# zeehu/generative_ranking_recommender

Measured on AMD Instinct MI355X. Metric: vectors quantized/sec (3-level RQ, 512-d), higher is better.
Workload: dtype f32

## Files before the change

generative_ranking_recommender_amd/csrc/assign_common.h:

```cpp
#pragma once
#include <cmath>
#include <cstdlib>
#include <type_traits>

#include "assign_plan.h"
#include "internal.h"

#ifndef RQSID_AB_MODE
#define RQSID_AB_MODE 0
#endif

namespace rqsid {

typedef __attribute__((ext_vector_type(8))) _Float16 f16x8;
typedef __attribute__((ext_vector_type(2))) _Float16 h2;
typedef __attribute__((ext_vector_type(2))) float f2;
typedef __attribute__((ext_vector_type(16))) float f32x16;

constexpr int kWaves = 4;
constexpr int kRowsPerWave = 32;
constexpr int kTileRows = kWaves * kRowsPerWave;
constexpr int kChunk = 32;
constexpr int kXWaveBytes = kRowsPerWave * 128;
constexpr int kXStage = kWaves * kXWaveBytes;
// ... 117 lines not shown
__device__ __forceinline__ void dma16_nt_off(const void* gsrc, uint32_t lds_base) {
  uint32_t keep;
  asm volatile(
      RQ_M0_SAVE
      "s_mov_b32 m0, %2\n\t"
      "s_nop 0\n\t"
      "global_load_lds_dwordx4 %1, off offset:%3 nt"
      RQ_M0_RESTORE
      : "=&s"(keep)
      : "v"(gsrc), "s"(lds_base), "i"(OFF)
      : "memory");
}
__device__ __forceinline__ void dma16_nt(const void* gsrc, uint32_t lds_base) {
  uint32_t keep;
  asm volatile(
      RQ_M0_SAVE
      "s_mov_b32 m0, %2\n\t"
      "s_nop 0\n\t"
      "global_load_lds_dwordx4 %1, off nt"
      RQ_M0_RESTORE
      : "=&s"(keep)
      : "v"(gsrc), "s"(lds_base)
      : "memory");
}

__device__ __forceinline__ void dma16_r(const void* gsrc, uint32_t lds_base) {
  uint32_t keep;
  asm volatile(
      RQ_M0_SAVE
      "s_mov_b32 m0, %2\n\t"
      "s_nop 0\n\t"
      "global_load_lds_dwordx4 %1, off"
      RQ_M0_RESTORE
      : "=&s"(keep)
      : "v"(gsrc), "s"(lds_base));
}
__device__ __forceinline__ void dma16_nt_r(const void* gsrc, uint32_t lds_base) {
  uint32_t keep;
  asm volatile(
      RQ_M0_SAVE
      "s_mov_b32 m0, %2\n\t"
      "s_nop 0\n\t"
      "global_load_lds_dwordx4 %1, off nt"
      RQ_M0_RESTORE
      : "=&s"(keep)
      : "v"(gsrc), "s"(lds_base));
}
#define RQSID_PIN_MFMA() __builtin_amdgcn_sched_barrier(0x0106)

template <int N>
__device__ __forceinline__ void wait_barrier() {
  asm volatile("s_waitcnt vmcnt(%0)\n\ts_waitcnt lgkmcnt(0)\n\ts_barrier" ::"i"(N) : "memory");
}

template <int S, int P>
__device__ __forceinline__ void wait_chunks(int younger) {
  static_assert((S - 2) * P <= 63, "vmcnt field is 6 bits");
  if (S >= 7 && younger >= 5) wait_barrier<(S >= 7 ? 5 * P : 0)>();
  else if (S >= 6 && younger >= 4) wait_barrier<(S >= 6 ? 4 * P : 0)>();
  else if (S >= 5 && younger >= 3) wait_barrier<(S >= 5 ? 3 * P : 0)>();
  else if (S >= 4 && younger >= 2) wait_barrier<(S >= 4 ? 2 * P : 0)>();
  else if (younger >= 1) wait_barrier<P>();
  else wait_barrier<0>();
}

__device__ __forceinline__ int xor32(int x) {
  const auto sw = __builtin_amdgcn_permlane32_swap((unsigned)x, (unsigned)x, false, false);
  return (int)((threadIdx.x & 32) ? sw[0] : sw[1]);
}
__device__ __forceinline__ float xor32(float x) { return __int_as_float(xor32(__float_as_int(x))); }
__device__ __forceinline__ double xor32(double x) {
  const uint64_t u = (uint64_t)__double_as_longlong(x);
  const uint64_t lo = (uint32_t)xor32((int)(uint32_t)u), hi = (uint32_t)xor32((int)(uint32_t)(u >> 32));
  return __longlong_as_double((long long)((hi << 32) | lo));
}

__device__ __forceinline__ void push_work(const AssignParams& p, bool need, int lane, const WorkItem& w) {
  const unsigned long long m = __ballot(need);
  if (!m) return;
  const int leader = __ffsll((long long)m) - 1;
  int base = 0;
  if (lane == leader) base = atomicAdd(p.work_count, __popcll(m));
  base = __shfl(base, leader);
  if (need) {
    const int idx = base + __popcll(m & ((1ull << lane) - 1ull));
    if (idx < p.work_cap) p.work[idx] = w;
  }
}

constexpr double kTrunc = 16.0;
inline float accumulation_rel(int dim) {
  return (float)((kTrunc + (dim / 16) / 2.0 + 1.0) * std::ldexp(1.0, -23) * 1.02);
}

template <int NW>
__device__ __forceinline__ int pass_take_first(uint32_t (&wv)[NW], int h) {
  int ws = -1;
  uint32_t b = 0;
#pragma unroll
  for (int w = NW - 1; w >= 0; --w) {
    const bool nz = wv[w] != 0;
    ws = nz ? w : ws;
    b = nz ? wv[w] : b;
  }
  const int jj = __clz(b) & 31;
  const int t = 2 * ws + (jj >> 4), v = jj & 15;
  const int k = ws >= 0 ? t * 32 + (v & 3) + 8 * (v >> 2) + 4 * h : -1;
#pragma unroll
  for (int w = 0; w < NW; ++w) wv[w] = w == ws ? (wv[w] & ~(0x80000000u >> jj)) : wv[w];
  return k;
}

template <int NW>
__device__ __forceinline__ bool pass_decide(const uint32_t (&pbits)[NW], int h, int& k_out, WorkItem& w) {
  int pc = 0;
#pragma unroll
  for (int i = 0; i < NW; ++i) pc += __popc(pbits[i]);
  const int pc_o = xor32(pc);
  const int ncand = pc + pc_o;
  const bool overflow = pc > kListPerHalf || pc_o > kListPerHalf || ncand == 0;
  const bool definitive = !overflow && ncand == 1;
  uint32_t wv[NW];
#pragma unroll
  for (int i = 0; i < NW; ++i) wv[i] = pbits[i];
  const int k0 = pass_take_first(wv, h);
  k_out = max(k0, xor32(k0));
  w.n = overflow ? -1 : ncand;
  if (__builtin_amdgcn_ballot_w64(!definitive && !overflow)) {
    int kk[kListPerHalf];
    kk[0] = k0;
#pragma unroll
    for (int j = 1; j < kListPerHalf; ++j) kk[j] = pass_take_first(wv, h);
    int c8[kMaxList];
#pragma unroll
    for (int j = 0; j < kListPerHalf; ++j) {
      const int o = xor32(kk[j]);
      c8[j] = kk[j] >= 0 ? kk[j] : INT_MAX;
      c8[kListPerHalf + j] = o >= 0 ? o : INT_MAX;
    }
#pragma unroll
    for (int i = 0; i < kMaxList; ++i)
#pragma unroll
      for (int j = 0; j < kMaxList - 1 - i; ++j) {
        const int a = c8[j], bq = c8[j + 1];
        c8[j] = min(a, bq);
        c8[j + 1] = max(a, bq);
      }
#pragma unroll
    for (int j = 0; j < kMaxList; ++j) w.cand[j] = (uint16_t)(c8[j] == INT_MAX ? 0xFFFF : c8[j]);
  }
  return definitive;
}

__device__ __forceinline__ float ratio_up(float num, float den) {
  return den > 0.f ? num / den * 1.000001f : (num > 0.f ? INFINITY : 0.f);
}
__device__ __forceinline__ float wave_max(float v) {
#pragma unroll
  for (int o = 32; o > 0; o >>= 1) v = fmaxf(v, __shfl_xor(v, o));
  return v;
}

#ifdef RQSID_STAMPS
#define ST_NOW() __builtin_amdgcn_s_memtime()
#define ST(x) x
#else
#define ST(x)
#endif

#ifndef RQSID_PACKED_MAIN
#define RQSID_PACKED_MAIN 0
#endif

constexpr int kErrSlot = 60;
constexpr int kErrCompact = 1;
constexpr int kErrOvfList = 2;
constexpr int kErrWorkIdx = 4;
constexpr int kErrTiles = 8;

struct RowSums {
  f2 se2v = {0.f, 0.f};
  f2 se2l = {0.f, 0.f};
  f2 sf2v = {0.f, 0.f};
  double sv2 = 0.0;
  double sv2b = 0.0;
};
constexpr bool fp64_norm(int rl, bool norm) { return norm && rl == 1; }

template <int HI>
__device__ __forceinline__ float sub_f16(float v, h2 hh) {
  float d;
  if (HI)
    asm("v_fma_mix_f32 %0, -%1, 1.0, %2 op_sel:[1,0,0] op_sel_hi:[1,0,0]" : "=v"(d) : "v"(hh), "v"(v));
  else
    asm("v_fma_mix_f32 %0, -%1, 1.0, %2 op_sel:[0,0,0] op_sel_hi:[1,0,0]" : "=v"(d) : "v"(hh), "v"(v));
  return d;
}

template <int XF, bool INFNAN>
__device__ __forceinline__ void widen2(uint32_t w, float& lo, float& hi) {
  static_assert(XF == RQSID_X_F16 || XF == RQSID_X_BF16, "16-bit row formats");
  if (XF == RQSID_X_BF16) {
    lo = __uint_as_float(w << 16);
    hi = __uint_as_float(w & 0xFFFF0000u);
  } else {
    const uint32_t sl = w << 16;
    uint32_t al = (w << 13) & 0x0FFFE000u, ah = (w >> 3) & 0x0FFFE000u;
    float fl = __uint_as_float(al) * 0x1p112f, fh = __uint_as_float(ah) * 0x1p112f;
    if (INFNAN) {
      fl = al >= 0x0F800000u ? __uint_as_float(__float_as_uint(fl) | 0x7F800000u) : fl;
      fh = ah >= 0x0F800000u ? __uint_as_float(__float_as_uint(fh) | 0x7F800000u) : fh;
    }
    lo = __uint_as_float((__float_as_uint(fl) & 0x7FFFFFFFu) | (sl & 0x80000000u));
    hi = __uint_as_float((__float_as_uint(fh) & 0x7FFFFFFFu) | (w & 0x80000000u));
  }
}
template <int XF>
__device__ __forceinline__ float4 load_row4(const float* x, int64_t row, int dim, int i) {
  if constexpr (XF == RQSID_X_F32) {
    return reinterpret_cast<const float4*>(x + row * dim)[i];
  } else {
    const uint2 w = reinterpret_cast<const uint2*>(reinterpret_cast<const uint16_t*>(x) + row * dim)[i];
    float4 a;
    widen2<XF, true>(w.x, a.x, a.y);
    widen2<XF, true>(w.y, a.z, a.w);
    return a;
  }
}

template <int RL, bool NORM, bool T3, bool SUMS>
__device__ __forceinline__ void row_frag(const float4 xa, const float4 xc, const float* lds_ca, const float* lds_cb,
                                         int d0, float inv1, f16x8& bf, f16x8& bl, RowSums& s) {
#if RQSID_PACKED_MAIN
  f2 v[4] = {f2{xa.x, xa.y}, f2{xa.z, xa.w}, f2{xc.x, xc.y}, f2{xc.z, xc.w}};
  if (RL >= 1) {
    const float4 a0 = *reinterpret_cast<const float4*>(lds_ca + d0);
    const float4 a1 = *reinterpret_cast<const float4*>(lds_ca + d0 + 4);
    const f2 av[4] = {f2{a0.x, a0.y}, f2{a0.z, a0.w}, f2{a1.x, a1.y}, f2{a1.z, a1.w}};
#pragma unroll
    for (int e = 0; e < 4; ++e) v[e] = v[e] - av[e];
  }
  if (RL >= 2) {
    const float4 b0 = *reinterpret_cast<const float4*>(lds_cb + d0);
    const float4 b1 = *reinterpret_cast<const float4*>(lds_cb + d0 + 4);
    const f2 bv[4] = {f2{b0.x, b0.y}, f2{b0.z, b0.w}, f2{b1.x, b1.y}, f2{b1.z, b1.w}};
#pragma unroll
    for (int e = 0; e < 4; ++e) v[e] = (NORM ? v[e] * inv1 : v[e]) - bv[e];
  }
  h2 hh[4], lh[4];
#pragma unroll
  for (int e = 0; e < 4; ++e) hh[e] = __builtin_convertvector(v[e], h2);
  bf = __builtin_shufflevector(__builtin_shufflevector(hh[0], hh[1], 0, 1, 2, 3),
                               __builtin_shufflevector(hh[2], hh[3], 0, 1, 2, 3), 0, 1, 2, 3, 4, 5, 6, 7);
  if (T3) {
#pragma unroll
    for (int e = 0; e < 4; ++e) {
      const f2 xs = (v[e] - __builtin_convertvector(hh[e], f2)) * 4096.0f;
      lh[e] = __builtin_convertvector(xs, h2);
      if (SUMS) {
        const f2 ev = xs - __builtin_convertvector(lh[e], f2);
        s.se2l = ev * ev + s.se2l;
      }
    }
    bl = __builtin_shufflevector(__builtin_shufflevector(lh[0], lh[1], 0, 1, 2, 3),
                                 __builtin_shufflevector(lh[2], lh[3], 0, 1, 2, 3), 0, 1, 2, 3, 4, 5, 6, 7);
  }
  if (SUMS) {
#pragma unroll
    for (int e = 0; e < 4; ++e) {
      const f2 ex = v[e] - __builtin_convertvector(hh[e], f2);
      s.se2v = ex * ex + s.se2v;
      if (fp64_norm(RL, NORM)) {
        s.sv2 = fma((double)v[e].x, (double)v[e].x, s.sv2);
        s.sv2b = fma((double)v[e].y, (double)v[e].y, s.sv2b);
      } else {
        s.sf2v = v[e] * v[e] + s.sf2v;
      }
    }
  }
#else
  float v[8] = {xa.x, xa.y, xa.z, xa.w, xc.x, xc.y, xc.z, xc.w};
  if (RL >= 1) {
    const float4 a0 = *reinterpret_cast<const float4*>(lds_ca + d0);
    const float4 a1 = *reinterpret_cast<const float4*>(lds_ca + d0 + 4);
    const float a[8] = {a0.x, a0.y, a0.z, a0.w, a1.x, a1.y, a1.z, a1.w};
#pragma unroll
    for (int e = 0; e < 8; ++e) v[e] = v[e] - a[e];
  }
  if (RL >= 2) {
    const float4 b0 = *reinterpret_cast<const float4*>(lds_cb + d0);
    const float4 b1 = *reinterpret_cast<const float4*>(lds_cb + d0 + 4);
    const float b[8] = {b0.x, b0.y, b0.z, b0.w, b1.x, b1.y, b1.z, b1.w};
#pragma unroll
    for (int e = 0; e < 8; ++e) v[e] = (NORM ? v[e] * inv1 : v[e]) - b[e];
  }
  h2 hh[4], lh[4];
#pragma unroll
  for (int e = 0; e < 4; ++e) hh[e] = __builtin_convertvector(f2{v[2 * e], v[2 * e + 1]}, h2);
  bf = __builtin_shufflevector(__builtin_shufflevector(hh[0], hh[1], 0, 1, 2, 3),
                               __builtin_shufflevector(hh[2], hh[3], 0, 1, 2, 3), 0, 1, 2, 3, 4, 5, 6, 7);
  float ex[8];
#pragma unroll
  for (int e = 0; e < 8; ++e) ex[e] = (e & 1) ? sub_f16<1>(v[e], hh[e >> 1]) : sub_f16<0>(v[e], hh[e >> 1]);
  if (T3) {
#pragma unroll
    for (int e = 0; e < 4; ++e) lh[e] = __builtin_convertvector(f2{ex[2 * e] * 4096.0f, ex[2 * e + 1] * 4096.0f}, h2);
// ... 99 lines not shown
```

generative_ranking_recommender_amd/csrc/assign_pc.hip:

```cpp
#define RQ_M0_KEEP 0
#include "assign_common.h"

#ifdef RQSID_STAMPS
__device__ unsigned long long g_pc_stamps[24];
#define PST(...) __VA_ARGS__
#define PNOW() __builtin_amdgcn_s_memtime()
#else
#define PST(...)
#endif

namespace rqsid {
namespace {

constexpr int kQDim = 512, kQC = 32, kQNch = kQDim / kQC;
constexpr int kQRows = 128;
constexpr int kQSentinel = -2;

struct PcDesc {
  int32_t s, t0, nrows, cnt, cbase, flags, ca_row, cb_row;
};
static_assert(sizeof(PcDesc) == 32, "descriptor layout");
static_assert(kQDim == kPlanPcDim && kQRows == kPlanPcRows && sizeof(PcDesc) == kPlanPcDescBytes, "assign_plan.h constants");

template <int NT, int RL, bool T3>
struct PcLayout {
  static constexpr int Sr = 4, Sc = 3;
  static constexpr int kTerms = T3 ? 2 : 1;
  static constexpr int kXS = kQRows * kQC * 4;
  static constexpr int kCT = NT * 32 * kQC * 2;
  static constexpr int kCS = kCT * kTerms;
  static constexpr int kBW = 2 * kTerms * 1024;
  static constexpr int kBS = 4 * kBW;
  static constexpr int kX = 0;
  static constexpr int kC = kX + Sr * kXS;
  static constexpr int kB = kC + Sc * kCS;
  static constexpr int kH = kB + 2 * kBS;
  static constexpr int kHRow = 0;
  static constexpr int kHCidx = kHRow + kQRows * 4;
  static constexpr int kHCsq = kHCidx + NT * 128;
  static constexpr int kHY = kHCsq + NT * 128;
  static constexpr int kHDen = kHY + NT * 128;
  static constexpr int kHRes = kHDen + kQRows * 4;
  static constexpr int kHBytes = kHRes + RL * kQDim * 4;
  static constexpr int kCoef = kH + 2 * kHBytes;
  static constexpr int kBytes = kCoef + kQRows * 16;
  static constexpr int kCI = NT / 2;
  static constexpr int H = 3;
  static_assert(kCI * kTerms == 4, "four centre DMA ops per loader and phase");
  static_assert(kBytes <= 160 * 1024, "LDS budget");
};

__device__ __forceinline__ int uni(int v) { return __builtin_amdgcn_readfirstlane(v); }
__device__ __forceinline__ uint64_t uni64(const void* ptr) {
  const uint64_t a = reinterpret_cast<uint64_t>(ptr);
  return ((uint64_t)__builtin_amdgcn_readfirstlane((uint32_t)(a >> 32)) << 32) |
         (uint32_t)__builtin_amdgcn_readfirstlane((uint32_t)a);
}
__device__ __forceinline__ PcDesc load_desc(const PcDesc* d) {
  typedef __attribute__((ext_vector_type(8))) int i32x8;
  i32x8 v;
  asm volatile("s_load_dwordx8 %0, %1, 0x0\n\ts_waitcnt lgkmcnt(0)" : "=s"(v) : "s"(uni64(d)) : "memory");
  PcDesc o;
  o.s = v[0]; o.t0 = v[1]; o.nrows = v[2]; o.cnt = v[3]; o.cbase = v[4]; o.flags = v[5]; o.ca_row = v[6]; o.cb_row = v[7];
  return o;
}
__device__ __forceinline__ void dma4(const void* gsrc, uint32_t lds_base) {
  uint32_t keep;
  asm volatile(
      RQ_M0_SAVE
      "s_mov_b32 m0, %2\n\t"
      "s_nop 0\n\t"
      "global_load_lds_dword %1, off"
      RQ_M0_RESTORE
      : "=&s"(keep)
      : "v"(gsrc), "s"(lds_base)
      : "memory");
}
template <int N>
__device__ __forceinline__ void vm_lgkm_barrier() {
  asm volatile("s_waitcnt vmcnt(%0)\n\ts_waitcnt lgkmcnt(0)\n\ts_barrier" ::"i"(N) : "memory");
}
__device__ __forceinline__ void lgkm_barrier() { asm volatile("s_waitcnt lgkmcnt(0)\n\ts_barrier" ::: "memory"); }

template <int NT, int RL, bool NORM, bool T3>
__global__ __launch_bounds__(768, 3) void assign_pc_kernel(AssignParams p, const int32_t* seg_tiles,
                                                           const PcDesc* desc) {
  using L = PcLayout<NT, RL, T3>;
  constexpr int kCI = L::kCI, H = L::H;
  extern __shared__ __attribute__((aligned(16))) unsigned char smem[];
  asm volatile("s_setreg_imm32_b32 hwreg(HW_REG_MODE, 6, 2), 0");
  const int tid = threadIdx.x, lane = tid & 63;
  const int wave = uni(tid >> 6);
  const int h = lane >> 5, r = lane & 31;
  const uint32_t lds0 = lds_addr(smem);

  const int ntiles = uni(seg_tiles[p.n_segments]);
  const int G8 = (int)(gridDim.x >> 3), xcd = (int)(blockIdx.x & 7), slot = (int)(blockIdx.x >> 3);
  const int xlo = (int)((int64_t)xcd * ntiles / 8), xhi = (int)((int64_t)(xcd + 1) * ntiles / 8);
  const int T0 = xlo + slot;
  if (T0 >= xhi) return;

  if (wave < 4) {
    const int c = wave;
    const int csw = (r >> 2) & 3;
    f32x16 acc[NT];
    f32x16 accl[T3 ? NT : 1];
    auto compute = [&](int g, bool first) __attribute__((always_inline)) {
      const f32x16 zero16 = {};
      const unsigned char* bimg = smem + L::kB + (g & 1) * L::kBS + c * L::kBW + lane * 16;
      const unsigned char* cimg0 = smem + L::kC + (g % L::Sc) * L::kCS + r * 64;
      f16x8 bf[2], bl[2];
#pragma unroll
      for (int ks = 0; ks < 2; ++ks) {
        bf[ks] = *reinterpret_cast<const f16x8*>(bimg + (ks * L::kTerms) * 1024);
        if (T3) bl[ks] = *reinterpret_cast<const f16x8*>(bimg + (ks * L::kTerms + 1) * 1024);
      }
#pragma unroll
      for (int ks = 0; ks < 2; ++ks) {
        const unsigned char* cimg = cimg0 + (((2 * ks + h) ^ csw) << 4);
#pragma unroll
        for (int t = 0; t < NT; ++t) {
          const f16x8 af = *reinterpret_cast<const f16x8*>(cimg + t * 32 * 64);
          acc[t] = __builtin_amdgcn_mfma_f32_32x32x16_f16(af, bf[ks], (first && ks == 0) ? zero16 : acc[t], 0, 0, 0);
          if (T3) {
            const f16x8 al = *reinterpret_cast<const f16x8*>(cimg + L::kCT + t * 32 * 64);
            accl[T3 ? t : 0] = __builtin_amdgcn_mfma_f32_32x32x16_f16(af, bl[ks], (first && ks == 0) ? zero16 : accl[T3 ? t : 0],
                                                                      0, 0, 0);
            accl[T3 ? t : 0] = __builtin_amdgcn_mfma_f32_32x32x16_f16(al, bf[ks], accl[T3 ? t : 0], 0, 0, 0);
          }
        }
      }
    };
    PST(uint64_t s_eM = 0, s_eU = 0, s_eB = 0, s_eD = 0;)
    auto epilogue = [&](const PcDesc& D, int par) __attribute__((always_inline)) {
#ifdef RQSID_STAMPS
      uint64_t e0 = PNOW();
      {
        float dmy;
        asm volatile("v_mov_b32 %0, %1" : "=v"(dmy) : "v"(acc[NT - 1][15]));
        asm volatile("s_waitcnt lgkmcnt(0)" ::"v"(dmy));
      }
      s_eM += PNOW() - e0;
      e0 = PNOW();
#endif
      const unsigned char* hb = smem + L::kH + par * L::kHBytes;
      const int lr = 32 * c + r;
      const bool row_valid = lr < D.nrows;
      const int my_row = p.row_index ? reinterpret_cast<const int*>(hb + L::kHRow)[min(lr, D.nrows - 1)]
                                     : D.t0 + min(lr, D.nrows - 1);
      auto cand_of = [&](int k) -> int {
        if (D.flags & 1) return 0;
        if (!p.cand_idx) return D.cbase + min(k, D.cnt - 1);
        return reinterpret_cast<const int*>(hb + L::kHCidx)[min(k, NT * 32 - 1)];
      };
      int out_l = kQSentinel, out_g = kQSentinel;
      bool need = false;
      WorkItem w{};
      w.row = my_row;
      w.seg = D.s;
      if (D.flags & 1) {
        need = true;
        w.n = (D.flags & 2) ? -2 : -3;
      } else {
        const float4 rc = *reinterpret_cast<const float4*>(smem + L::kCoef + lr * 16);
        const f2 m2v = {rc.x, rc.x}, a2v = {rc.y, rc.y}, na2v = {-rc.y, -rc.y};
        const float* m_csq = reinterpret_cast<const float*>(hb + L::kHCsq);
        const float* m_y = reinterpret_cast<const float*>(hb + L::kHY);
        float U = INFINITY;
#pragma unroll
        for (int t = 0; t < NT; ++t) {
#pragma unroll
          for (int gq = 0; gq < 4; ++gq) {
            const float4 csq = *reinterpret_cast<const float4*>(m_csq + t * 32 + 8 * gq + 4 * h);
            const float4 yy = *reinterpret_cast<const float4*>(m_y + t * 32 + 8 * gq + 4 * h);
#pragma unroll
            for (int e = 0; e < 2; ++e) {
              const int v = 4 * gq + 2 * e;
              f2 d = {acc[t][v], acc[t][v + 1]};
              if (T3) d = f2{accl[T3 ? t : 0][v], accl[T3 ? t : 0][v + 1]} * 0x1p-12f + d;
              const f2 P2 = m2v * d + (e ? f2{csq.z, csq.w} : f2{csq.x, csq.y});
              const f2 y2 = e ? f2{yy.z, yy.w} : f2{yy.x, yy.y};
              const f2 ub = a2v * y2 + P2, lb = na2v * y2 + P2;
              U = fminf(U, fminf(ub.x, ub.y));
              acc[t][v] = lb.x;
              acc[t][v + 1] = lb.y;
            }
          }
        }
        U = fminf(U, xor32(U));
        const float Up = fmaf(fabsf(U), 0x1p-22f, U) + (1.2e-38f + 2e-30f);
        PST(asm volatile("" ::"v"(Up)); s_eU += PNOW() - e0; e0 = PNOW();)
        const f2 upv = {Up, Up};
        uint32_t pbt[NT];
#pragma unroll
        for (int t = 0; t < NT; ++t) pbt[t] = 0u;
#pragma unroll
        for (int v = 0; v < 16; v += 2)
#pragma unroll
          for (int t = 0; t < NT; ++t) {
            const f2 d = f2{acc[t][v], acc[t][v + 1]} - upv;
            pbt[t] = __builtin_amdgcn_alignbit(pbt[t], __float_as_uint(d.x), 31);
            pbt[t] = __builtin_amdgcn_alignbit(pbt[t], __float_as_uint(d.y), 31);
          }
        uint32_t pbits[NT / 2];
#pragma unroll
        for (int wd = 0; wd < NT / 2; ++wd) pbits[wd] = (pbt[2 * wd] << 16) | pbt[2 * wd + 1];
        if (D.cnt < NT * 32) {
#pragma unroll
          for (int wd = 0; wd < NT / 2; ++wd) {
            uint32_t m = 0;
#pragma unroll
            for (int qq = 0; qq < 2; ++qq) {
              const int rem = D.cnt - 32 * (2 * wd + qq) - 4 * h;
              int nv = 0;
#pragma unroll
              for (int gq = 0; gq < 4; ++gq) nv += min(4, max(0, rem - 8 * gq));
              const uint32_t pre = (uint32_t)((0xFFFFull << (16 - nv)) & 0xFFFFull);
              m |= qq == 0 ? pre << 16 : pre;
            }
            pbits[wd] &= m;
          }
        }
        PST(asm volatile("" ::"v"(pbits[0]), "v"(pbits[NT / 2 - 1])); s_eB += PNOW() - e0; e0 = PNOW();)
        int k = -1;
        if (pass_decide(pbits, h, k, w)) {
          out_l = p.cand_lid ? cand_local(p, D.cbase, k) : k;
          out_g = cand_of(k);
        } else {
          need = true;
        }
      }
      if (h == 0 && row_valid) {
        p.out_local[my_row] = out_l;
        p.out_global[my_row] = out_g;
        if (need) p.work[my_row] = w;
        if (RL == 1 && NORM) p.den_out[my_row] = reinterpret_cast<const float*>(smem + L::kCoef + lr * 16)[2];
      }
      PST(s_eD += PNOW() - e0;)
    };
    lgkm_barrier();
    lgkm_barrier();
    lgkm_barrier();
    PST(uint64_t s_bar = 0, s_cmp = 0, s_epi = 0; const uint64_t s_t0 = PNOW(); uint64_t s_a;)
    int g = 0;
    for (int T = T0; T < xhi; T += G8) {
      const int par = (g >> 4) & 1;
      PST(s_a = PNOW();)
      compute(g, true);
      const PcDesc D = load_desc(desc + T);
      PST(s_cmp += PNOW() - s_a; s_a = PNOW();)
      lgkm_barrier();
      PST(s_bar += PNOW() - s_a;)
      ++g;
#pragma unroll 1
      for (int j = 1; j < kQNch - 1; ++j, ++g) {
        PST(s_a = PNOW();)
        compute(g, false);
        PST(s_cmp += PNOW() - s_a; s_a = PNOW();)
        lgkm_barrier();
        PST(s_bar += PNOW() - s_a;)
      }
      PST(s_a = PNOW();)
      compute(g, false);
      PST(s_cmp += PNOW() - s_a; s_a = PNOW();)
      epilogue(D, par);
      PST(s_epi += PNOW() - s_a; s_a = PNOW();)
      lgkm_barrier();
      PST(s_bar += PNOW() - s_a;)
      ++g;
    }
#ifdef RQSID_STAMPS
    if (lane == 0) {
      atomicAdd(&g_pc_stamps[0], (unsigned long long)(PNOW() - s_t0));
      atomicAdd(&g_pc_stamps[1], (unsigned long long)s_bar);
      atomicAdd(&g_pc_stamps[3], (unsigned long long)s_epi);
      atomicAdd(&g_pc_stamps[4], 1ull);
      atomicAdd(&g_pc_stamps[5], (unsigned long long)s_cmp);
      atomicAdd(&g_pc_stamps[2], (unsigned long long)s_eM);
      atomicAdd(&g_pc_stamps[6], (unsigned long long)s_eU);
      atomicAdd(&g_pc_stamps[7], (unsigned long long)s_eB);
      atomicAdd(&g_pc_stamps[23], (unsigned long long)s_eD);
    }
#endif
    return;
  }

  const float* trow = p.c_meta + 4 * (int64_t)p.n_centers;
  auto hdr_base = [&](int par) { return lds0 + L::kH + par * L::kHBytes; };
  auto row_of = [&](const PcDesc& D, int par, int lr) -> int {
    const int l = min(lr, D.nrows - 1);
    return p.row_index ? reinterpret_cast<const int*>(smem + L::kH + par * L::kHBytes + L::kHRow)[l] : D.t0 + l;
  };

  if (wave < 8) {
    const int q = wave - 4;
    const float tscale = __uint_as_float(uni(__float_as_uint(trow[0])));
    const float tgz = __uint_as_float(uni(__float_as_uint(trow[1])));
    const float tgw = __uint_as_float(uni(__float_as_uint(trow[2])));
    const float tgy = __uint_as_float(uni(__float_as_uint(trow[3])));
    const int xsw = (r >> 1) & 7;
    const char* const xbase = reinterpret_cast<const char*>(p.x);
    struct XSrc {
      uint64_t xo[4];
    };
    auto x_src = [&](const PcDesc& D, int par, XSrc& s) {
#pragma unroll
      for (int i = 0; i < 4; ++i) {
        const int lr = 8 * i + (lane >> 3);
        const int sl = (lane & 7) ^ ((lr >> 1) & 7);
        s.xo[i] = (uint64_t)(uint32_t)row_of(D, par, 32 * q + lr) * 2048u + (uint64_t)(sl * 16);
      }
    };
    auto issue_r = [&](const XSrc& s, int cj, int st) {
      const uint32_t sx = lds0 + L::kX + st * L::kXS + q * 4096;
      const char* xb = xbase + cj * (kQC * 4);
#pragma unroll
      for (int i = 0; i < 4; ++i) dma16_nt(xb + s.xo[i], uni(sx + i * 1024));
    };
    RowSums rs;
    float inv1 = 1.0f;
    auto build = [&](const PcDesc& D, int par, int cj, int rst, int bst) {
      const unsigned char* hb = smem + L::kH + par * L::kHBytes;
      if (cj == 0) {
        rs = RowSums{};
        if (RL == 2 && NORM) inv1 = 1.0f / reinterpret_cast<const float*>(hb + L::kHDen)[32 * q + r];
      }
      const float* lds_ca = reinterpret_cast<const float*>(hb + L::kHRes);
      const float* lds_cb = reinterpret_cast<const float*>(hb + L::kHRes + (RL == 2 ? kQDim * 4 : 0));
      const unsigned char* xrow = smem + L::kX + rst * L::kXS + q * 4096 + r * 128;
      unsigned char* bimg = smem + L::kB + bst * L::kBS + q * L::kBW + lane * 16;
#pragma unroll
      for (int ks = 0; ks < 2; ++ks) {
        const int q0 = 4 * ks + 2 * h;
        const float4 xa = *reinterpret_cast<const float4*>(xrow + ((q0 ^ xsw) << 4));
        const float4 xc = *reinterpret_cast<const float4*>(xrow + (((q0 + 1) ^ xsw) << 4));
        f16x8 bf, bl = {};
        row_frag<RL, NORM, T3, true>(xa, xc, lds_ca, lds_cb, cj * kQC + 16 * ks + 8 * h, inv1, bf, bl, rs);
        *reinterpret_cast<f16x8*>(bimg + (ks * L::kTerms) * 1024) = bf;
        if (T3) *reinterpret_cast<f16x8*>(bimg + (ks * L::kTerms + 1) * 1024) = bl;
      }
    };
    auto finish = [&]() {
      const int lr = 32 * q + r;
      float inv_den = 1.f, dr = 0.f, vn, en, en2 = 0.f, den = 0.f;
      const float se2 = rs.se2v.x + rs.se2v.y, sf2 = rs.sf2v.x + rs.sf2v.y;
      en = sqrtf(se2 + xor32(se2)) * 1.001f + 1e-30f;
      if (T3) {
        const float l2 = rs.se2l.x + rs.se2l.y;
        en2 = sqrtf(l2 + xor32(l2)) * (1.001f / 4096.0f) + 1e-30f;
      }
      float nrm;
      if (NORM && RL >= 1) {
        if (RL == 1) {
          const double t2 = rs.sv2 + rs.sv2b;
          nrm = (float)sqrt(t2 + xor32(t2));
        } else {
          nrm = sqrtf(sf2 + xor32(sf2));
        }
        den = nrm + 1e-8f;
        inv_den = 1.0f / den;
        const float den_eps = (0.125f * (float)(kQDim) + 3.0f) * 5.97e-8f;
        dr = RL == 1 ? 2.0f * 5.97e-8f
                     : (4.0f * 2.39e-7f * (1.0f + nrm) * inv_den + 4.0f * 5.97e-8f + 1.01f * den_eps * nrm * inv_den);
      } else {
        nrm = sqrtf(sf2 + xor32(sf2));
      }
      vn = nrm * 1.0001f + 1e-30f;
      const float hn = vn + en;
      const float vr = vn * inv_den;
      const float ar = p.acc_rel, ar2 = 2.0f * p.acc_rel, k2 = 2.0f * inv_den * 1.000001f;
      const float A = T3 ? k2 * (en2 + ar * hn + ar2 * (en + en2)) + 2.0f * dr + 7.2e-7f * vr
                         : k2 * (en + ar * hn) + 2.0f * dr + 4.8e-7f * vr;
      const float B = T3 ? k2 * (hn * (1.0f + ar2) + 2.0f * (en + en2)) : k2 * hn * (1.0f + ar);
      const float C = T3 ? k2 * ((en + en2) + ar * hn + ar2 * (hn + en + en2)) : 0.0f;
      const float m2 = -2.0f * inv_den * tscale;
      const float A2 = (A + B * (T3 ? tgz : tgw) + C * tgw + 2.39e-7f * tgy) * 1.000001f;
      if (h == 0) *reinterpret_cast<float4*>(smem + L::kCoef + lr * 16) = make_float4(m2, A2, den, 0.f);
    };

    PcDesc Dc = load_desc(desc + T0);
    lgkm_barrier();
    XSrc cur, nxt;
    x_src(Dc, 0, cur);
#pragma unroll
    for (int i = 0; i < 4; ++i) issue_r(cur, i, i);
    vm_lgkm_barrier<0>();
    build(Dc, 0, 0, 0, 0);
    lgkm_barrier();
    PcDesc Dn = Dc;
    PST(uint64_t s_bar = 0, s_vm = 0, s_fin = 0, s_bld = 0, s_iss = 0; const uint64_t s_t0 = PNOW(); uint64_t s_a;)
    int g = 0;
    for (int T = T0; T < xhi; T += G8) {
      const int Tn = T + G8;
      const bool more = Tn < xhi;
      const int par = (g >> 4) & 1;
#pragma unroll 1
      for (int j = 0; j < kQNch; ++j, ++g) {
        PST(s_a = PNOW();)
        {
          const int cj = j + 4;
          issue_r(cj < kQNch ? cur : nxt, cj & (kQNch - 1), (g + 4) & 3);
        }
        PST(s_iss += PNOW() - s_a;)
        if (j == 0) Dn = load_desc(desc + (more ? Tn : T));
        if (j == 4) x_src(Dn, par ^ 1, nxt);
        PST(s_a = PNOW();)
        asm volatile("s_waitcnt vmcnt(12)" ::: "memory");
        PST(s_vm += PNOW() - s_a; s_a = PNOW();)
        if (j < kQNch - 1) build(Dc, par, j + 1, (g + 1) & 3, (g + 1) & 1);
        else build(Dn, par ^ 1, 0, (g + 1) & 3, (g + 1) & 1);
        PST(s_bld += PNOW() - s_a; s_a = PNOW();)
        if (j == kQNch - 2) finish();
        PST(s_fin += PNOW() - s_a; s_a = PNOW();)
        lgkm_barrier();
        PST(s_bar += PNOW() - s_a;)
      }
      Dc = Dn;
      cur = nxt;
    }
    asm volatile("s_waitcnt vmcnt(0)" ::: "memory");
#ifdef RQSID_STAMPS
    if (lane == 0) {
      atomicAdd(&g_pc_stamps[8], (unsigned long long)(PNOW() - s_t0));
      atomicAdd(&g_pc_stamps[9], (unsigned long long)s_bar);
      atomicAdd(&g_pc_stamps[10], (unsigned long long)s_vm);
      atomicAdd(&g_pc_stamps[11], (unsigned long long)s_fin);
      atomicAdd(&g_pc_stamps[12], 1ull);
      atomicAdd(&g_pc_stamps[13], (unsigned long long)s_bld);
      atomicAdd(&g_pc_stamps[14], (unsigned long long)s_iss);
    }
#endif
    return;
  }

  const int q = wave - 8;
  const bool hi_tab = !T3 && p.c16h;
  const char* const cbase16 = reinterpret_cast<const char*>(hi_tab ? p.c16h : p.c16);
  const uint32_t cunits = hi_tab ? 64u : 128u;
  const int cchunk = hi_tab ? kQC * 2 : kQC * 4;
  struct CSrc {
    uint32_t ci[kCI];
  };
  auto hdr_level1 = [&](const PcDesc& D, int par) {
    const int lr = min(32 * q + r, D.nrows - 1);
    if (lane < 32)
      dma4(p.row_index ? (const void*)(p.row_index + D.t0 + lr) : (const void*)p.seg_row_off,
           uni(hdr_base(par) + L::kHRow + q * 128));
    const int k = q * (NT * 8) + (lane & (NT * 8 - 1));
    const int kc = D.cnt > 0 ? min(k, D.cnt - 1) : 0;
    if (NT == 8 || lane < 32)
      dma4(p.cand_idx && D.cnt > 0 ? (const void*)(p.cand_idx + D.cbase + kc) : (const void*)p.seg_row_off,
           uni(hdr_base(par) + L::kHCidx + q * (NT * 32)));
    const bool second = RL == 2 && q >= 2;
    const int half = q & 1;
    const float* src = second ? p.cb + (int64_t)D.cb_row * kQDim : p.ca + (int64_t)D.ca_row * kQDim;
    dma16(src + half * 256 + lane * 4, uni(hdr_base(par) + L::kHRes + (second ? kQDim * 4 : 0) + half * 1024));
  };
  auto cand_of = [&](const PcDesc& D, int par, int k) -> int {
    if (D.flags & 1) return 0;
    if (!p.cand_idx) return D.cbase + min(k, D.cnt - 1);
    return reinterpret_cast<const int*>(smem + L::kH + par * L::kHBytes + L::kHCidx)[min(k, NT * 32 - 1)];
  };
  auto c_src = [&](const PcDesc& D, int par, CSrc& s) {
#pragma unroll
    for (int j = 0; j < kCI; ++j) {
      const int k = (q * kCI + j) * 16 + (lane >> 2);
      const int sl = (lane & 3) ^ ((k >> 2) & 3);
      s.ci[j] = (uint32_t)cand_of(D, par, k) * cunits + (uint32_t)sl;
    }
  };
  auto hdr_level2 = [&](const PcDesc& D, int par) {
    const int k = q * (NT * 8) + (lane & (NT * 8 - 1));
    const float* m = p.c_meta + 4 * (int64_t)cand_of(D, par, k);
    if (NT == 8 || lane < 32) {
      dma4(m, uni(hdr_base(par) + L::kHCsq + q * (NT * 32)));
      dma4(m + 1, uni(hdr_base(par) + L::kHY + q * (NT * 32)));
    }
    if (lane < 32)
      dma4(RL == 2 && NORM ? (const void*)(p.den_in + row_of(D, par, 32 * q + r)) : (const void*)p.seg_row_off,
           uni(hdr_base(par) + L::kHDen + q * 128));
  };
  auto issue_c = [&](const CSrc& s, int cj, int st) {
    const uint32_t sc = lds0 + L::kC + st * L::kCS;
    const char* cb = cbase16 + cj * cchunk;
#pragma unroll
    for (int j = 0; j < kCI; ++j) dma16(cb + (uint64_t)s.ci[j] * 16u, uni(sc + (q * kCI + j) * 1024));
    if (T3) {
#pragma unroll
      for (int j = 0; j < kCI; ++j) dma16(cb + kQC * 2 + (uint64_t)s.ci[j] * 16u, uni(sc + L::kCT + (q * kCI + j) * 1024));
    }
  };

  PcDesc Dc = load_desc(desc + T0);
  hdr_level1(Dc, 0);
  vm_lgkm_barrier<0>();
  CSrc cur, nxt;
  c_src(Dc, 0, cur);
  hdr_level2(Dc, 0);
  issue_c(cur, 0, 0);
  issue_c(cur, 1, 1);
  vm_lgkm_barrier<0>();
  lgkm_barrier();
  PcDesc Dn = Dc;
  PST(uint64_t s_bar = 0, s_vm = 0, s_iss = 0; const uint64_t s_t0 = PNOW(); uint64_t s_a;)
  int g = 0;
  for (int T = T0; T < xhi; T += G8) {
    const int Tn = T + G8;
    const bool more = Tn < xhi;
    const int par = (g >> 4) & 1;
#pragma unroll 1
    for (int j = 0; j < kQNch; ++j, ++g) {
      PST(s_a = PNOW();)
      {
        const int cj = j + 2;
        issue_c(cj < kQNch ? cur : nxt, cj & (kQNch - 1), (g + 2) % L::Sc);
      }
      PST(s_iss += PNOW() - s_a;)
      if (j == 0) Dn = load_desc(desc + (more ? Tn : T));
      if (j == 1) hdr_level1(Dn, par ^ 1);
      if (j == 4) {
        c_src(Dn, par ^ 1, nxt);
        hdr_level2(Dn, par ^ 1);
      }
      PST(s_a = PNOW();)
#ifdef RQSID_STAMPS
      if (j == 1 || j == 2 || j == 4 || j == 5) asm volatile("s_waitcnt vmcnt(%0)" ::"i"(kCI * L::kTerms + H) : "memory");
      else asm volatile("s_waitcnt vmcnt(%0)" ::"i"(kCI * L::kTerms) : "memory");
      s_vm += PNOW() - s_a;
      s_a = PNOW();
#endif
// ... 491 lines not shown
```

Baseline: 600.8 million.

## Transpose MFMA operands so rows map to lanes and centres to accumulator registers in epilogue

Swaps the A/B operands of the MFMA so each lane's accumulator holds one centre across several rows, rather than one row across several centres. The epilogue is rewritten around this: per-row coefficients move to a struct-of-arrays LDS layout, row minima are reduced across the half-wave with DPP and permlane16_swap, and pass bitmasks are built per row with ballots plus v_writelane. Candidate lists are then extracted by popcount/ffs over the bit words. The goal is cheaper bound computation and candidate selection per row, paid for with more cross-lane traffic and hand-written inline asm.

```diff
diff --git a/generative_ranking_recommender_amd/csrc/assign_common.h b/generative_ranking_recommender_amd/csrc/assign_common.h
--- a/generative_ranking_recommender_amd/csrc/assign_common.h
+++ b/generative_ranking_recommender_amd/csrc/assign_common.h
@@ -293,6 +293,69 @@
   return definitive;
 }
 
+template <int NW>
+__device__ __forceinline__ int pass_take_lowest(uint32_t (&wv)[NW]) {
+  int ws = -1;
+  uint32_t b = 0;
+#pragma unroll
+  for (int w = NW - 1; w >= 0; --w) {
+    const bool nz = wv[w] != 0;
+    ws = nz ? w : ws;
+    b = nz ? wv[w] : b;
+  }
+  const int k = ws >= 0 ? 32 * ws + (__ffs((int)b) - 1) : -1;
+#pragma unroll
+  for (int w = 0; w < NW; ++w) wv[w] = w == ws ? (b & (b - 1u)) : wv[w];
+  return k;
+}
+template <int NW>
+__device__ __forceinline__ bool pass_decide_words(const uint32_t (&pw)[NW], int& k_out, WorkItem& w) {
+  int pc = 0;
+#pragma unroll
+  for (int i = 0; i < NW; ++i) pc += __popc(pw[i]);
+  const bool overflow = pc > kMaxList || pc == 0;
+  const bool definitive = pc == 1;
+  uint32_t wv[NW];
+#pragma unroll
+  for (int i = 0; i < NW; ++i) wv[i] = pw[i];
+  k_out = pass_take_lowest(wv);
+  w.n = overflow ? -1 : pc;
+  const bool listed = !definitive && !overflow;
+  if (__builtin_amdgcn_ballot_w64(listed)) {
+    w.cand[0] = (uint16_t)(k_out >= 0 ? k_out : 0xFFFF);
+#pragma unroll
+    for (int j = 1; j < kMaxList; ++j) w.cand[j] = 0xFFFF;
+#pragma unroll
+    for (int j = 1; j < kMaxList; ++j) {
+      if (!__builtin_amdgcn_ballot_w64(listed && pc > j)) break;
+      const int k = pass_take_lowest(wv);
+      w.cand[j] = (uint16_t)(k >= 0 ? k : 0xFFFF);
+    }
+  }
+  return definitive;
+}
+
+__device__ __forceinline__ void half_min4(float& a, float& b, float& c, float& d) {
+  float ta, tb, tc, td;
+#define RQ_MIN4(ctl)                                                  \
+  "v_min_f32_dpp %0, %0, %0 " ctl " row_mask:0xf bank_mask:0xf\n\t"   \
+  "v_min_f32_dpp %1, %1, %1 " ctl " row_mask:0xf bank_mask:0xf\n\t"   \
+  "v_min_f32_dpp %2, %2, %2 " ctl " row_mask:0xf bank_mask:0xf\n\t"   \
+  "v_min_f32_dpp %3, %3, %3 " ctl " row_mask:0xf bank_mask:0xf\n\t"
+  asm volatile(
+      "s_nop 1\n\t"
+      RQ_MIN4("quad_perm:[1,0,3,2]")
+      RQ_MIN4("quad_perm:[2,3,0,1]")
+      RQ_MIN4("row_half_mirror")
+      RQ_MIN4("row_mirror")
+      "v_mov_b32 %4, %0\n\tv_mov_b32 %5, %1\n\tv_mov_b32 %6, %2\n\tv_mov_b32 %7, %3\n\t"
+      "v_permlane16_swap_b32 %4, %0\n\tv_permlane16_swap_b32 %5, %1\n\t"
+      "v_permlane16_swap_b32 %6, %2\n\tv_permlane16_swap_b32 %7, %3\n\t"
+      "v_min_f32 %0, %0, %4\n\tv_min_f32 %1, %1, %5\n\tv_min_f32 %2, %2, %6\n\tv_min_f32 %3, %3, %7"
+      : "+v"(a), "+v"(b), "+v"(c), "+v"(d), "=&v"(ta), "=&v"(tb), "=&v"(tc), "=&v"(td));
+#undef RQ_MIN4
+}
+
 __device__ __forceinline__ float ratio_up(float num, float den) {
   return den > 0.f ? num / den * 1.000001f : (num > 0.f ? INFINITY : 0.f);
 }
diff --git a/generative_ranking_recommender_amd/csrc/assign_pc.hip b/generative_ranking_recommender_amd/csrc/assign_pc.hip
--- a/generative_ranking_recommender_amd/csrc/assign_pc.hip
+++ b/generative_ranking_recommender_amd/csrc/assign_pc.hip
@@ -43,6 +43,7 @@
   static constexpr int kHRes = kHDen + kQRows * 4;
   static constexpr int kHBytes = kHRes + RL * kQDim * 4;
   static constexpr int kCoef = kH + 2 * kHBytes;
+  static constexpr int kCoefA2 = kQRows * 4, kCoefDen = 2 * kQRows * 4;
   static constexpr int kBytes = kCoef + kQRows * 16;
   static constexpr int kCI = NT / 2;
   static constexpr int H = 3;
@@ -76,6 +77,37 @@
       : "v"(gsrc), "s"(lds_base)
       : "memory");
 }
+template <int LANE>
+__device__ __forceinline__ void write_lanes(uint32_t (&v)[8], const uint64_t (&m)[8]) {
+#define RQ_L(t) (uint32_t)m[t]
+#define RQ_H(t) (uint32_t)(m[t] >> 32)
+  asm volatile(
+      "s_nop 1\n\t"
+      "v_writelane_b32 %0, %8, %24\n\tv_writelane_b32 %1, %9, %24\n\tv_writelane_b32 %2, %10, %24\n\t"
+      "v_writelane_b32 %3, %11, %24\n\tv_writelane_b32 %4, %12, %24\n\tv_writelane_b32 %5, %13, %24\n\t"
+      "v_writelane_b32 %6, %14, %24\n\tv_writelane_b32 %7, %15, %24\n\t"
+      "v_writelane_b32 %0, %16, %25\n\tv_writelane_b32 %1, %17, %25\n\tv_writelane_b32 %2, %18, %25\n\t"
+      "v_writelane_b32 %3, %19, %25\n\tv_writelane_b32 %4, %20, %25\n\tv_writelane_b32 %5, %21, %25\n\t"
+      "v_writelane_b32 %6, %22, %25\n\tv_writelane_b32 %7, %23, %25"
+      : "+v"(v[0]), "+v"(v[1]), "+v"(v[2]), "+v"(v[3]), "+v"(v[4]), "+v"(v[5]), "+v"(v[6]), "+v"(v[7])
+      : "s"(RQ_L(0)), "s"(RQ_L(1)), "s"(RQ_L(2)), "s"(RQ_L(3)), "s"(RQ_L(4)), "s"(RQ_L(5)), "s"(RQ_L(6)), "s"(RQ_L(7)),
+        "s"(RQ_H(0)), "s"(RQ_H(1)), "s"(RQ_H(2)), "s"(RQ_H(3)), "s"(RQ_H(4)), "s"(RQ_H(5)), "s"(RQ_H(6)), "s"(RQ_H(7)),
+        "n"(LANE), "n"(LANE + 4));
+}
+template <int LANE>
+__device__ __forceinline__ void write_lanes(uint32_t (&v)[4], const uint64_t (&m)[4]) {
+  asm volatile(
+      "s_nop 1\n\t"
+      "v_writelane_b32 %0, %4, %12\n\tv_writelane_b32 %1, %5, %12\n\tv_writelane_b32 %2, %6, %12\n\t"
+      "v_writelane_b32 %3, %7, %12\n\t"
+      "v_writelane_b32 %0, %8, %13\n\tv_writelane_b32 %1, %9, %13\n\tv_writelane_b32 %2, %10, %13\n\t"
+      "v_writelane_b32 %3, %11, %13"
+      : "+v"(v[0]), "+v"(v[1]), "+v"(v[2]), "+v"(v[3])
+      : "s"(RQ_L(0)), "s"(RQ_L(1)), "s"(RQ_L(2)), "s"(RQ_L(3)), "s"(RQ_H(0)), "s"(RQ_H(1)), "s"(RQ_H(2)), "s"(RQ_H(3)),
+        "n"(LANE), "n"(LANE + 4));
+#undef RQ_L
+#undef RQ_H
+}
 template <int N>
 __device__ __forceinline__ void vm_lgkm_barrier() {
   asm volatile("s_waitcnt vmcnt(%0)\n\ts_waitcnt lgkmcnt(0)\n\ts_barrier" ::"i"(N) : "memory");
@@ -102,11 +134,17 @@
 
   if (wave < 4) {
     const int c = wave;
-    const int csw = (r >> 2) & 3;
+    auto lane_now = [&]() __attribute__((always_inline)) {
+      int ln;
+      asm volatile("v_mbcnt_lo_u32_b32 %0, -1, 0\n\tv_mbcnt_hi_u32_b32 %0, -1, %0" : "=v"(ln));
+      return ln;
+    };
     f32x16 acc[NT];
     f32x16 accl[T3 ? NT : 1];
     auto compute = [&](int g, bool first) __attribute__((always_inline)) {
       const f32x16 zero16 = {};
+      const int lane = lane_now(), h = lane >> 5, r = lane & 31;
+      const int csw = (r >> 2) & 3;
       const unsigned char* bimg = smem + L::kB + (g & 1) * L::kBS + c * L::kBW + lane * 16;
       const unsigned char* cimg0 = smem + L::kC + (g % L::Sc) * L::kCS + r * 64;
       f16x8 bf[2], bl[2];
@@ -121,17 +159,17 @@
 #pragma unroll
         for (int t = 0; t < NT; ++t) {
           const f16x8 af = *reinterpret_cast<const f16x8*>(cimg + t * 32 * 64);
-          acc[t] = __builtin_amdgcn_mfma_f32_32x32x16_f16(af, bf[ks], (first && ks == 0) ? zero16 : acc[t], 0, 0, 0);
+          acc[t] = __builtin_amdgcn_mfma_f32_32x32x16_f16(bf[ks], af, (first && ks == 0) ? zero16 : acc[t], 0, 0, 0);
           if (T3) {
             const f16x8 al = *reinterpret_cast<const f16x8*>(cimg + L::kCT + t * 32 * 64);
-            accl[T3 ? t : 0] = __builtin_amdgcn_mfma_f32_32x32x16_f16(af, bl[ks], (first && ks == 0) ? zero16 : accl[T3 ? t : 0],
+            accl[T3 ? t : 0] = __builtin_amdgcn_mfma_f32_32x32x16_f16(bl[ks], af, (first && ks == 0) ? zero16 : accl[T3 ? t : 0],
                                                                       0, 0, 0);
-            accl[T3 ? t : 0] = __builtin_amdgcn_mfma_f32_32x32x16_f16(al, bf[ks], accl[T3 ? t : 0], 0, 0, 0);
+            accl[T3 ? t : 0] = __builtin_amdgcn_mfma_f32_32x32x16_f16(bf[ks], al, accl[T3 ? t : 0], 0, 0, 0);
           }
         }
       }
     };
-    PST(uint64_t s_eM = 0, s_eU = 0, s_eB = 0, s_eD = 0;)
+    PST(uint64_t s_eM = 0, s_eU = 0, s_eB = 0, s_eD = 0, s_g1 = 0, s_g2 = 0, s_g3 = 0;)
     auto epilogue = [&](const PcDesc& D, int par) __attribute__((always_inline)) {
 #ifdef RQSID_STAMPS
       uint64_t e0 = PNOW();
@@ -144,10 +182,6 @@
       e0 = PNOW();
 #endif
       const unsigned char* hb = smem + L::kH + par * L::kHBytes;
-      const int lr = 32 * c + r;
-      const bool row_valid = lr < D.nrows;
-      const int my_row = p.row_index ? reinterpret_cast<const int*>(hb + L::kHRow)[min(lr, D.nrows - 1)]
-                                     : D.t0 + min(lr, D.nrows - 1);
       auto cand_of = [&](int k) -> int {
         if (D.flags & 1) return 0;
         if (!p.cand_idx) return D.cbase + min(k, D.cnt - 1);
@@ -156,85 +190,108 @@
       int out_l = kQSentinel, out_g = kQSentinel;
       bool need = false;
       WorkItem w{};
-      w.row = my_row;
-      w.seg = D.s;
       if (D.flags & 1) {
         need = true;
         w.n = (D.flags & 2) ? -2 : -3;
       } else {
-        const float4 rc = *reinterpret_cast<const float4*>(smem + L::kCoef + lr * 16);
-        const f2 m2v = {rc.x, rc.x}, a2v = {rc.y, rc.y}, na2v = {-rc.y, -rc.y};
-        const float* m_csq = reinterpret_cast<const float*>(hb + L::kHCsq);
-        const float* m_y = reinterpret_cast<const float*>(hb + L::kHY);
-        float U = INFINITY;
-#pragma unroll
-        for (int t = 0; t < NT; ++t) {
-#pragma unroll
-          for (int gq = 0; gq < 4; ++gq) {
-            const float4 csq = *reinterpret_cast<const float4*>(m_csq + t * 32 + 8 * gq + 4 * h);
-            const float4 yy = *reinterpret_cast<const float4*>(m_y + t * 32 + 8 * gq + 4 * h);
-#pragma unroll
-            for (int e = 0; e < 2; ++e) {
-              const int v = 4 * gq + 2 * e;
-              f2 d = {acc[t][v], acc[t][v + 1]};
-              if (T3) d = f2{accl[T3 ? t : 0][v], accl[T3 ? t : 0][v + 1]} * 0x1p-12f + d;
-              const f2 P2 = m2v * d + (e ? f2{csq.z, csq.w} : f2{csq.x, csq.y});
-              const f2 y2 = e ? f2{yy.z, yy.w} : f2{yy.x, yy.y};
-              const f2 ub = a2v * y2 + P2, lb = na2v * y2 + P2;
-              U = fminf(U, fminf(ub.x, ub.y));
-              acc[t][v] = lb.x;
-              acc[t][v + 1] = lb.y;
+        const int lane = lane_now(), h = lane >> 5, r = lane & 31;
+        const float* m_csq = reinterpret_cast<const float*>(hb + L::kHCsq) + r;
+        const float* m_y = reinterpret_cast<const float*>(hb + L::kHY) + r;
+        f2 cy[NT];
+#pragma unroll
+        for (int t = 0; t < NT; ++t) cy[t] = f2{m_csq[t * 32], m_y[t * 32]};
+#pragma unroll
+        for (int t = 0; t < NT; t += 4)
+          asm("" : "+v"(cy[t]), "+v"(cy[t + 1]), "+v"(cy[t + 2]), "+v"(cy[t + 3]));
+        const unsigned char* coef = smem + L::kCoef + (32 * c + 4 * h) * 4;
+        float4 m2q = *reinterpret_cast<const float4*>(coef);
+        float4 a2q = *reinterpret_cast<const float4*>(coef + L::kCoefA2);
+        uint32_t pw[NT];
+#pragma unroll
+        for (int t = 0; t < NT; ++t) pw[t] = 0u;
+#pragma unroll
+        for (int gq = 0; gq < 4; ++gq) {
+          PST(uint64_t g0 = PNOW();)
+          float U[4] = {INFINITY, INFINITY, INFINITY, INFINITY};
+#pragma unroll
+          for (int e = 0; e < 2; ++e) {
+            const f2 m2v = e ? f2{m2q.z, m2q.w} : f2{m2q.x, m2q.y};
+            const f2 a2v = e ? f2{a2q.z, a2q.w} : f2{a2q.x, a2q.y};
+            const f2 na2v = -a2v;
+            const int v = 4 * gq + 2 * e;
+#pragma unroll
+            for (int t = 0; t < NT; t += 2) {
+              f2 ub[2];
+#pragma unroll
+              for (int u = 0; u < 2; ++u) {
+                f2 d = {acc[t + u][v], acc[t + u][v + 1]};
+                if (T3) d = f2{accl[T3 ? t + u : 0][v], accl[T3 ? t + u : 0][v + 1]} * 0x1p-12f + d;
+                const f2 P2 = m2v * d + __builtin_shufflevector(cy[t + u], cy[t + u], 0, 0);
+                const f2 y2 = __builtin_shufflevector(cy[t + u], cy[t + u], 1, 1);
+                const f2 lb = na2v * y2 + P2;
+                ub[u] = a2v * y2 + P2;
+                acc[t + u][v] = lb.x;
+                acc[t + u][v + 1] = lb.y;
+              }
+              U[2 * e] = fminf(U[2 * e], fminf(ub[0].x, ub[1].x));
+              U[2 * e + 1] = fminf(U[2 * e + 1], fminf(ub[0].y, ub[1].y));
+              __builtin_amdgcn_sched_barrier(0);
             }
           }
+          if (gq < 3) {
+            m2q = *reinterpret_cast<const float4*>(coef + (gq + 1) * 32);
+            a2q = *reinterpret_cast<const float4*>(coef + L::kCoefA2 + (gq + 1) * 32);
+          }
+          __builtin_amdgcn_sched_barrier(0);
+          PST(asm volatile("" ::"v"(U[0]), "v"(U[3])); s_g1 += PNOW() - g0; g0 = PNOW();)
+          half_min4(U[0], U[1], U[2], U[3]);
+          PST(asm volatile("" ::"v"(U[0]), "v"(U[3])); s_g2 += PNOW() - g0; g0 = PNOW();)
+          auto pass_words = [&](auto I) __attribute__((always_inline)) {
+            constexpr int i = decltype(I)::value;
+            const float Up = fmaf(fabsf(U[i]), 0x1p-22f, U[i]) + (1.2e-38f + 2e-30f);
+            uint64_t m[NT];
+#pragma unroll
+            for (int t = 0; t < NT; ++t) m[t] = __builtin_amdgcn_ballot_w64(acc[t][4 * gq + i] < Up);
+            switch (gq) {
+              case 0: write_lanes<i>(pw, m); break;
+              case 1: write_lanes<8 + i>(pw, m); break;
+              case 2: write_lanes<16 + i>(pw, m); break;
+              default: write_lanes<24 + i>(pw, m); break;
+            }
+          };
+          pass_words(std::integral_constant<int, 0>());
+          pass_words(std::integral_constant<int, 1>());
+          pass_words(std::integral_constant<int, 2>());
+          pass_words(std::integral_constant<int, 3>());
+          PST(asm volatile("" ::"v"(pw[0]), "v"(pw[NT - 1])); s_g3 += PNOW() - g0;)
+          __builtin_amdgcn_sched_barrier(0);
         }
-        U = fminf(U, xor32(U));
-        const float Up = fmaf(fabsf(U), 0x1p-22f, U) + (1.2e-38f + 2e-30f);
-        PST(asm volatile("" ::"v"(Up)); s_eU += PNOW() - e0; e0 = PNOW();)
-        const f2 upv = {Up, Up};
-        uint32_t pbt[NT];
-#pragma unroll
-        for (int t = 0; t < NT; ++t) pbt[t] = 0u;
-#pragma unroll
-        for (int v = 0; v < 16; v += 2)
+        PST(asm volatile("" ::"v"(pw[0]), "v"(pw[NT - 1])); s_eU += PNOW() - e0; e0 = PNOW();)
+        if (D.cnt < NT * 32) {
 #pragma unroll
           for (int t = 0; t < NT; ++t) {
-            const f2 d = f2{acc[t][v], acc[t][v + 1]} - upv;
-            pbt[t] = __builtin_amdgcn_alignbit(pbt[t], __float_as_uint(d.x), 31);
-            pbt[t] = __builtin_amdgcn_alignbit(pbt[t], __float_as_uint(d.y), 31);
-          }
-        uint32_t pbits[NT / 2];
-#pragma unroll
-        for (int wd = 0; wd < NT / 2; ++wd) pbits[wd] = (pbt[2 * wd] << 16) | pbt[2 * wd + 1];
-        if (D.cnt < NT * 32) {
-#pragma unroll
-          for (int wd = 0; wd < NT / 2; ++wd) {
-            uint32_t m = 0;
-#pragma unroll
-            for (int qq = 0; qq < 2; ++qq) {
-              const int rem = D.cnt - 32 * (2 * wd + qq) - 4 * h;
-              int nv = 0;
-#pragma unroll
-              for (int gq = 0; gq < 4; ++gq) nv += min(4, max(0, rem - 8 * gq));
-              const uint32_t pre = (uint32_t)((0xFFFFull << (16 - nv)) & 0xFFFFull);
-              m |= qq == 0 ? pre << 16 : pre;
-            }
-            pbits[wd] &= m;
+            const int nv = min(32, max(0, D.cnt - 32 * t));
+            pw[t] &= (uint32_t)((1ull << nv) - 1ull);
           }
         }
-        PST(asm volatile("" ::"v"(pbits[0]), "v"(pbits[NT / 2 - 1])); s_eB += PNOW() - e0; e0 = PNOW();)
+        PST(asm volatile("" ::"v"(pw[0]), "v"(pw[NT - 1])); s_eB += PNOW() - e0; e0 = PNOW();)
         int k = -1;
-        if (pass_decide(pbits, h, k, w)) {
+        if (pass_decide_words(pw, k, w)) {
           out_l = p.cand_lid ? cand_local(p, D.cbase, k) : k;
           out_g = cand_of(k);
         } else {
           need = true;
         }
       }
-      if (h == 0 && row_valid) {
+      const int lr = 32 * c + lane_now();
+      if (lr < min(32 * c + 32, D.nrows)) {
+        const int my_row = p.row_index ? reinterpret_cast<const int*>(hb + L::kHRow)[lr] : D.t0 + lr;
+        w.row = my_row;
+        w.seg = D.s;
         p.out_local[my_row] = out_l;
         p.out_global[my_row] = out_g;
         if (need) p.work[my_row] = w;
-        if (RL == 1 && NORM) p.den_out[my_row] = reinterpret_cast<const float*>(smem + L::kCoef + lr * 16)[2];
+        if (RL == 1 && NORM) p.den_out[my_row] = reinterpret_cast<const float*>(smem + L::kCoef + L::kCoefDen)[lr];
       }
       PST(s_eD += PNOW() - e0;)
     };
@@ -280,6 +337,9 @@
       atomicAdd(&g_pc_stamps[6], (unsigned long long)s_eU);
       atomicAdd(&g_pc_stamps[7], (unsigned long long)s_eB);
       atomicAdd(&g_pc_stamps[23], (unsigned long long)s_eD);
+      atomicAdd(&g_pc_stamps[15], (unsigned long long)s_g1);
+      atomicAdd(&g_pc_stamps[19], (unsigned long long)s_g2);
+      atomicAdd(&g_pc_stamps[21], (unsigned long long)s_g3);
     }
 #endif
     return;
@@ -375,7 +435,11 @@
       const float C = T3 ? k2 * ((en + en2) + ar * hn + ar2 * (hn + en + en2)) : 0.0f;
       const float m2 = -2.0f * inv_den * tscale;
       const float A2 = (A + B * (T3 ? tgz : tgw) + C * tgw + 2.39e-7f * tgy) * 1.000001f;
-      if (h == 0) *reinterpret_cast<float4*>(smem + L::kCoef + lr * 16) = make_float4(m2, A2, den, 0.f);
+      if (h == 0) {
+        reinterpret_cast<float*>(smem + L::kCoef)[lr] = m2;
+        reinterpret_cast<float*>(smem + L::kCoef + L::kCoefA2)[lr] = A2;
+        reinterpret_cast<float*>(smem + L::kCoef + L::kCoefDen)[lr] = den;
+      }
     };
 
     PcDesc Dc = load_desc(desc + T0);
```

After: 608.4 million, median of 6. 1.01x the previous value.
